# pashtari/factorizer

Measured on AMD Instinct MI355X. Metric: volumes/sec fwd+bwd, Swin Factorizer 128^3, higher is better.
Workload: dtype f32

## Files before the change

### factorizer_amd/_native.py

```python
from __future__ import annotations

import ctypes
import os
import threading

import torch

_HERE = os.path.dirname(os.path.abspath(__file__))
LIB_PATH = os.environ.get("FZ_LIB_PATH") or os.path.join(_HERE, "libfactorizer_hip.so")

FZ_OK = 0
FZ_E_UNSUPPORTED = -2
ABI_VERSION = 7
SOLVER_ID = {"mu": 0, "hals": 1, "cd": 2, "smu": 3}
STORE_F32, STORE_BF16 = 0, 1
PRODUCTS_DEFAULT, PRODUCTS_SPLIT_BF16, PRODUCTS_FP32_MFMA = 0, 1, 2
_products = threading.local()


def products() -> int:
    return getattr(_products, "value", PRODUCTS_DEFAULT)


class use_products:
# ... 163 lines not shown
    _fields_ = [("p", _vp), ("M", _i), ("pmul", _vp), ("pmul_kind", _i), ("q", _vp * 4), ("nsrc", _i),
                ("src_mode", _i), ("c0", _i), ("Cin", _i), ("K", _i), ("Vq", _i64), ("D", _i), ("H", _i),
                ("W", _i), ("N", _i64), ("Ho", _i), ("Wo", _i), ("stats", _vp), ("qact", _i), ("ln_g", _vp),
                ("ln_b", _vp), ("gw", _vp), ("gbias", _vp), ("accumulate", _i), ("B", _i), ("loader", _i),
                ("act_dtype", _i), ("products", _i)]


class VolGeom(_c.Structure):
    _fields_ = [("nd", _i), ("size", _i * 3), ("start", _i * 3), ("end", _i * 3), ("pad", _i * 3), ("out", _i * 3)]


class RespaceGeom(_c.Structure):
    _fields_ = [("nd", _i), ("src_size", _i * 3), ("src_axis", _i * 3), ("flip", _i * 3), ("res_size", _i * 3), ("pad", _i * 3),
                ("out", _i * 3), ("orig_size", _i * 3), ("box_start", _i * 3), ("scale", _c.c_double * 3),
                ("inv_scale", _c.c_double * 3)]


_SIGS.update({
    "fz_gcorr_supported": ([_i] * 5, _i),
    "fz_gcorr": ([_vp] * 5 + [_i] * 11 + [_f, _vp], _i),
    "fz_gcorr_wgrad_workspace_bytes": ([_i] * 10, _i64),
    "fz_gcorr_wgrad": ([_vp] * 4 + [_i] * 11 + [_vp], _i),
    "fz_gcorr_act": ([_vp] * 5 + [_i] * 11 + [_f, _i, _vp], _i),
    "fz_gcorr_wgrad_act": ([_vp] * 4 + [_i] * 12 + [_vp], _i),
    "fz_gcorr_mu_bwd": ([_vp] * 8 + [_i] * 11 + [_f, _i, _vp], _i),
    "fz_gnmf_supported": ([_i, _i64, _i, _i, _i], _i),
    "fz_gnmf_workspace_bytes": ([_i64, _i, _i64, _i, _i, _i], _i64),
    "fz_gnmf_launches": ([_i, _i, _i], _i),
    "fz_gnmf_fwd": ([_vp] * 6 + [_i64, _i, _i64, _i, _i, _i, _f, _vp, _vp], _i),
    "fz_gnmf_bwd": ([_vp] * 7 + [_i64, _i, _i64, _i, _i, _i, _i, _f, _vp, _vp], _i),
    "fz_nmf_cf_supported": ([_i] * 11, _i),
    "fz_nmf_cf_fwd": ([_vp] * 4 + [_i] * 5 + [_c.POINTER(_i)] + [_i] * 5 + [_f, _i, _vp], _i),
    "fz_nmf_cf_bwd": ([_vp] * 5 + [_i] * 5 + [_c.POINTER(_i)] + [_i] * 7 + [_f, _i, _vp], _i),
    "fz_nmf_cf_factors_supported": ([_i] * 12 + [_c.POINTER(_i)], _i),
    "fz_nmf_cf_fwd_store_factors": ([_vp] * 5 + [_i] * 5 + [_c.POINTER(_i)] + [_i] * 3 + [_f, _i, _vp], _i),
    "fz_nmf_cf_fwd_from_factors": ([_vp] * 6 + [_i] * 5 + [_c.POINTER(_i)] * 2 + [_i] * 4 + [_f, _i, _vp], _i),
    "fz_nmf_cf_bwd_factors_supported": ([_i] * 14 + [_c.POINTER(_i)], _i),
    "fz_nmf_cf_bwd_store_factors": ([_vp] * 5 + [_i] * 5 + [_c.POINTER(_i)] + [_i] * 3 + [_f, _i, _vp], _i),
    "fz_nmf_cf_bwd_from_factors": ([_vp] * 6 + [_i] * 5 + [_c.POINTER(_i)] * 2 + [_i] * 3 + [_f, _i, _vp], _i),
    "fz_nmf_pcf_supported": ([_i] * 11, _i),
    "fz_nmf_pcf_fwd": ([_vp] * 4 + [_i] * 8 + [_c.POINTER(_i)] + [_i] * 5 + [_f, _i, _vp], _i),
    "fz_nmf_pcf_bwd": ([_vp] * 5 + [_i] * 8 + [_c.POINTER(_i)] + [_i] * 7 + [_f, _i, _vp], _i),
    "fz_nmf_pcf_bwd_prefers_separate": ([_i] * 4, _i),
    "fz_act_add": ([_vp, _vp, _i64, _i, _vp], _i),
    "fz_mlp_pre_supported": ([_i, _i, _i64, _i], _i),
    "fz_mlp_drop_supported": ([_i, _i, _i64, _i], _i),
    "fz_mlp_chain_drop": ([_c.POINTER(MlpDesc), _c.POINTER(MlpDropout), _vp], _i),
    "fz_conv3_prologue_supported": ([_i] * 4, _i),
    "fz_conv3_fwd2": ([_vp] * 4 + [_i] * 8 + [_c.POINTER(BlockPrologue), _vp], _i),
    "fz_upcat2": ([_vp, _vp, _vp, _i, _vp, _vp, _vp] + [_i] * 7 + [_c.POINTER(BlockPrologue), _vp], _i),
    "fz_gemm": ([_c.POINTER(GemmDesc), _vp], _i),
    "fz_gemm_bx_enable": ([_i], _i),
    "fz_gemm_lnbwd_partials": ([_c.POINTER(GemmDesc)], _i64),
    "fz_reduce_rows": ([_vp, _i64, _i, _vp, _vp, _vp], _i),
    "fz_adamw_step": ([_vp, _vp, _vp, _vp, _i64, _f, _f, _f, _f, _f, _i, _f, _vp], _i),
    "fz_sw_gather": ([_vp, _vp] + [_i] * 10 + [_vp], _i),
    "fz_sw_accumulate": ([_vp] * 6 + [_f] + [_i] * 10 + [_vp], _i),
    "fz_sw_finalize": ([_vp, _vp, _i, _i64, _vp], _i),
    "fz_sw_gather2": ([_vp, _vp] + [_i] * 11 + [_vp], _i),
    "fz_sw_accumulate2": ([_vp] * 6 + [_f] + [_i] * 11 + [_vp], _i),
    "fz_sw_finalize2": ([_vp, _vp, _vp, _i, _i64, _i, _vp], _i),
    "fz_mlp_supported": ([_i, _i, _i64], _i),
    "fz_mlp_partials": ([_i, _i64], _i64),
    "fz_mlp_wgrad_rows": ([_i, _i64], _i),
    "fz_gemm_dw_rows": ([_i, _i64], _i),
    "fz_gemm_dw_workspace_bytes": ([_i, _i64], _i64),
    "fz_gemm_dw": ([_c.POINTER(GemmDwDesc), _vp], _i),
    "fz_mlp_wgrad_workspace_bytes": ([_i, _i64], _i64),
    "fz_mlp_chain": ([_c.POINTER(MlpDesc), _vp], _i),
    "fz_head_bwd_rows": ([], _i),
    "fz_head_bwd_workspace_bytes": ([], _i64),
    "fz_head_bwd": ([_vp, _vp, _vp, _vp, _vp, _i, _i, _i, _i64, _i, _vp], _i),
    "fz_head_fwd": ([_vp, _vp, _vp, _vp, _i, _i, _i, _i64, _i, _vp], _i),
    "fz_upcat_supported": ([_i] * 5, _i),
    "fz_upcat_compose": ([_vp, _vp, _i, _vp, _vp, _vp, _vp, _vp, _i, _i, _i, _vp], _i),
    "fz_upcat_wgrads": ([_vp, _vp, _vp, _i, _vp, _vp, _vp, _vp, _i, _vp, _i, _i, _i, _vp], _i),
    "fz_upcat": ([_vp, _vp, _vp, _i, _vp, _vp, _vp] + [_i] * 7 + [_vp], _i),
    "fz_upcat_bwd_supported": ([_i] * 6, _i),
    "fz_upcat_bwd_workspace_bytes": ([_i] * 4, _i64),
    "fz_upcat_bwd": ([_vp, _vp, _vp, _vp, _i, _vp, _vp, _vp, _vp, _vp, _i, _vp, _vp] + [_i] * 7 + [_vp], _i),
    "fz_wgrad": ([_c.POINTER(WgradDesc), _vp, _vp], _i),
    "fz_wgrad_group": ([_c.POINTER(_c.POINTER(WgradDesc)), _c.POINTER(_vp), _i, _vp], _i),
    "fz_wgrad_workspace_bytes": ([_c.POINTER(WgradDesc)], _i64),
    "fz_conv3_fwd": ([_vp] * 4 + [_i] * 8 + [_vp], _i),
    "fz_conv3_wgrad_chunks": ([_i] * 4, _i),
    "fz_conv3_wgrad_partials": ([_vp] * 4 + [_i] * 8 + [_vp], _i),
    "fz_chunk_reduce": ([_vp, _i, _i64, _vp, _i, _vp], _i),
    "fz_chunk_reduce_ld": ([_vp, _i, _i64, _i64, _vp, _i, _vp], _i),
    "fz_finish_defer": ([_i], _i),
    "fz_finish_pending": ([], _i),
    "fz_finish_flush": ([_vp], _i),
    "fz_finish_flush_all": ([_vp], _i),
    "fz_dice_bce_chunks": ([_i64], _i),
    "fz_dice_bce_sums": ([_vp, _vp, _vp, _i, _i64, _vp], _i),
    "fz_dice_bce_grad": ([_vp, _vp, _vp, _vp, _i, _i64, _f, _f, _vp, _vp], _i),
    "fz_dice_ce_sums": ([_vp, _vp, _vp, _i, _i, _i64, _vp], _i),
    "fz_dice_ce_grad": ([_vp, _vp, _vp, _vp, _i, _i, _i64, _f, _f, _vp, _vp], _i),
    "fz_dice_ce_finish": ([_vp, _i, _i, _i64, _f, _vp, _vp, _vp], _i),
    "fz_dice_bce_ds_sums": ([_vp, _vp, _vp, _i] + [_i] * 6 + [_i, _vp], _i),
    "fz_dice_bce_ds_grad": ([_vp, _vp, _vp, _vp, _i] + [_i] * 6 + [_i, _f, _f, _vp, _vp], _i),
    "fz_dice_ce_ds_sums": ([_vp, _vp, _vp, _i, _i] + [_i] * 6 + [_i, _vp], _i),
    "fz_dice_ce_ds_grad": ([_vp, _vp, _vp, _vp, _i, _i] + [_i] * 6 + [_i, _f, _f, _vp, _vp], _i),
    "fz_rowsum_chunks": ([_i64], _i),
    "fz_rowsum": ([_vp, _vp, _vp, _i, _i, _i64, _i, _vp], _i),
    "fz_ln_fwd": ([_vp] * 5 + [_i, _i, _i64, _f, _i, _vp], _i),
    "fz_ln_bwd": ([_vp] * 8 + [_i, _i, _i64, _i, _vp], _i),
    "fz_ln_bwd_workspace_bytes": ([_i], _i64),
    "fz_ln_bwd_workspace_bytes2": ([_i, _i, _i64], _i64),
    "fz_dropout_bits_words": ([_i, _i, _i64], _i64),
    "fz_dropout_keep_bits": ([_vp, _i, _i, _i, _i64, _f, _vp, _vp], _i),
    "fz_dropout_apply": ([_i, _vp, _f, _vp, _vp, _vp, _i, _i, _i64, _i, _vp], _i),
    "fz_seg_counts_chunks": ([_i64], _i),
    "fz_seg_counts_workspace_bytes": ([_i, _i64], _i64),
    "fz_seg_counts": ([_vp, _i, _vp, _i, _f, _vp, _vp, _vp, _i, _i64, _vp], _i),
    "fz_mask_edges": ([_vp, _vp, _vp, _i, _i, _i, _i, _i, _vp], _i),
    "fz_edge_min_dist2_splits": ([_i64, _i64], _i),
    "fz_edge_min_dist2_workspace_bytes": ([_i64, _i64], _i64),
    "fz_edge_min_dist2": ([_vp, _i64, _vp, _i64, _f, _f, _f, _vp, _vp, _vp], _i),
    "fz_aug_record_floats": ([], _i),
    "fz_aug_resample": ([_vp, _vp, _i, _i, _vp, _vp, _i, _vp, _vp, _vp] + [_i] * 6 + [_vp], _i),
    "fz_aug_smooth": ([_vp, _vp, _i, _i, _vp, _vp] + [_i] * 6 + [_vp], _i),
    "fz_aug_noise_field": ([_vp, _vp, _i, _i, _i64, _vp], _i),
    "fz_aug_source_words": ([], _i),
    "fz_aug_crop_resample": ([_vp, _vp, _i, _i, _vp, _i, _vp, _vp, _vp] + [_i] * 6 + [_vp], _i),
    "fz_vol_kind_ok": ([_i, _i], _i),
    "fz_vol_bbox": ([_vp, _i, _i, _i, _i, _i, _i, _vp, _vp], _i),
    "fz_vol_workspace_bytes": ([_i, _c.POINTER(VolGeom)], _i64),
    "fz_vol_stats": ([_vp, _i, _i, _c.POINTER(VolGeom), _i, _i, _vp, _vp], _i),
    "fz_vol_write": ([_vp, _i, _vp, _i, _i, _vp, _i, _i, _c.POINTER(_i), _c.POINTER(_i), _i, _vp, _c.POINTER(VolGeom), _i, _i,
                      _vp, _vp, _vp, _vp], _i),
    "fz_vol_restore": ([_c.POINTER(_vp), _i, _i, _i, _c.POINTER(VolGeom), _f, _c.POINTER(_c.c_ubyte), _vp, _vp], _i),
    "fz_vol_respace": ([_vp, _i, _vp, _i, _vp, _i, _vp, _c.POINTER(RespaceGeom), _i, _vp], _i),
    "fz_vol_unspace": ([_c.POINTER(_vp), _i, _i, _i, _c.POINTER(RespaceGeom), _i, _i, _f, _vp, _vp], _i),
    "fz_inorm_one_pass_max": ([], _i),
    "fz_inorm_chunks": ([_i64], _i),
    "fz_inorm_workspace_bytes": ([_i64, _i64], _i64),
    "fz_inorm_fwd": ([_vp] * 5 + [_i64, _i, _i64, _c.c_double, _i, _vp, _vp], _i),
    "fz_inorm_bwd": ([_vp] * 7 + [_i64, _i, _i64, _i, _vp, _vp], _i),
})
SEG_F32, SEG_BF16, SEG_U8 = 0, 1, 2
VOL_F32, VOL_BF16, VOL_U8, VOL_I16 = 0, 1, 2, 3
VOL_IMAGE_IN, VOL_IMAGE_OUT, VOL_LABEL_IN, VOL_LOGITS = 0, 1, 2, 3
RESPACE_BILINEAR, RESPACE_NEAREST = 0, 1
DROP_RES, DROP_GELU, DROP_GELU_BWD = 0, 1, 2
```

### factorizer_amd/csrc/wgrad.hip

```cpp
#include <type_traits>

#include "fz_common.h"
#include "finish.h"

namespace fz {

typedef float f32x16 __attribute__((ext_vector_type(16)));
typedef float f32x2 __attribute__((ext_vector_type(2)));
typedef __bf16 bf16x2 __attribute__((ext_vector_type(2)));
typedef __bf16 bf16x8 __attribute__((ext_vector_type(8)));

__device__ __forceinline__ void split_bf16x8(const float (&x)[8], bf16x8& hi, bf16x8& mid, bf16x8& lo) {
#pragma unroll
  for (int e = 0; e < 8; e += 2) {
    const f32x2 v = {x[e], x[e + 1]};
    const bf16x2 h2 = __builtin_convertvector(v, bf16x2);
    const f32x2 r = v - __builtin_convertvector(h2, f32x2);
    const bf16x2 m2 = __builtin_convertvector(r, bf16x2);
    const f32x2 r2 = r - __builtin_convertvector(m2, f32x2);
    const bf16x2 l2 = __builtin_convertvector(r2, bf16x2);
    hi[e] = h2[0]; hi[e + 1] = h2[1];
    mid[e] = m2[0]; mid[e + 1] = m2[1];
    lo[e] = l2[0]; lo[e + 1] = l2[1];
  }
// ... 262 lines not shown
    for (int i = 0; i < MBP; ++i) {
      float s = psum[i] + __shfl_xor(psum[i], 32, 64);
      if (h == 0) red[wave * 32 + c] = s;
      __syncthreads();
      if (threadIdx.x < 32) {
        const float tot = (red[threadIdx.x] + red[32 + threadIdx.x]) + (red[64 + threadIdx.x] + red[96 + threadIdx.x]);
        const int m = m0 + i * 32 + threadIdx.x;
        if (m < a.M) a.part_bias[(int64_t)blockIdx.x * a.M + m] = tot;
      }
      __syncthreads();
    }
  }
}

enum { QP_NONE = 0, QP_STATS = 1, QP_GELU = 2, QP_RELU = 3 };
constexpr int kStrideF = 36;

template <int MBP, int MBQ, int QPRO, int BF, typename AT>
__device__ __forceinline__ void wgrad_fast_body(const WgradArgsT<AT>& a, float* lds, const int bx, const int by, const int bz) {
#define WG_BX bx
#define WG_BY by
#define WG_BZ bz
#include "wgrad_fast_body.inc"
#undef WG_BX
#undef WG_BY
#undef WG_BZ
}

template <int MBP, int MBQ, int QPRO, int BF = 0, typename AT = float>
__global__ __launch_bounds__(256, 2) void wgrad_fast_kernel(WgradArgsT<AT> a) {
  extern __shared__ __attribute__((aligned(16))) float lds[];
#define WG_BX blockIdx.x
#define WG_BY blockIdx.y
#define WG_BZ blockIdx.z
#include "wgrad_fast_body.inc"
#undef WG_BX
#undef WG_BY
#undef WG_BZ
}

constexpr int kWgGroupMax = 4;
template <typename AT>
struct WgradGroupT {
  WgradArgsT<AT> a[kWgGroupMax];
  int start[kWgGroupMax + 1];
  int gx[kWgGroupMax], gy[kWgGroupMax];
  int qpro[kWgGroupMax];
  int n;
};

template <int MBP, int MBQ, int BF, typename AT>
__global__ __launch_bounds__(256, 2) void wgrad_fast_group_kernel(WgradGroupT<AT> g) {
  extern __shared__ __attribute__((aligned(16))) float lds[];
  int i = 0;
#pragma unroll
  for (int t = 1; t < kWgGroupMax; ++t)
    if (t < g.n && (int)blockIdx.x >= g.start[t]) i = t;
  int local = (int)blockIdx.x - g.start[i];
  const int bx = local % g.gx[i];
  local /= g.gx[i];
  const int by = local % g.gy[i], bz = local / g.gy[i];
  const WgradArgsT<AT>& a = g.a[i];
  switch (g.qpro[i]) {
    case QP_STATS: wgrad_fast_body<MBP, MBQ, QP_STATS, BF, AT>(a, lds, bx, by, bz); break;
    case QP_GELU: wgrad_fast_body<MBP, MBQ, QP_GELU, BF, AT>(a, lds, bx, by, bz); break;
    case QP_RELU: wgrad_fast_body<MBP, MBQ, QP_RELU, BF, AT>(a, lds, bx, by, bz); break;
    default: wgrad_fast_body<MBP, MBQ, QP_NONE, BF, AT>(a, lds, bx, by, bz); break;
  }
}


__global__ __launch_bounds__(256) void ln_fold_kernel(float* __restrict__ gw, const float* __restrict__ acc,
                                                      const float* __restrict__ gb, const float* __restrict__ ln_g,
                                                      const float* __restrict__ ln_b, int M, int K, int accumulate) {
  const int64_t e = (int64_t)blockIdx.x * blockDim.x + threadIdx.x;
  if (e >= (int64_t)M * K) return;
  const int m = (int)(e / K), k = (int)(e % K);
  const float v = ln_g[k] * acc[e] + ln_b[k] * gb[m];
  gw[e] = accumulate ? gw[e] + v : v;
}

}

using namespace fz;

static bool use_fast(const fz_wgrad_desc* d) {
  const int PR = d->M > 32 ? 64 : 32, QR = d->K > 32 ? 64 : 32;
  const int c0 = d->c0 > 0 ? d->c0 : d->Cin;
  bool fast = PR == 64 && QR == 64 && d->loader == QL_PLAIN && !d->pmul && (d->M % PR) == 0 && (d->K % QR) == 0 &&
              (d->N % kTile) == 0 && d->N == d->Vq && (c0 % 8) == 0 && d->src_mode == 0 && !(d->stats && d->qact) &&
              (int64_t)8 * d->N < ((int64_t)1 << 30);
  { const auto& k = FZ_KNOB("FZ_WGRAD_FAST"); if (k.set && k.val == 0) fast = false; }
  return fast;
}

static int pick_chunks(int64_t total_tiles, int out_blocks, bool fast, int* tiles_per_chunk) {
  int64_t total_units = fast ? 1024 : 2048;
  int64_t units_target = total_units / (out_blocks > 0 ? out_blocks : 1);
  if (units_target < 16) units_target = 16;
  int64_t tpc = (total_tiles + units_target - 1) / units_target;
  if (tpc < 1) tpc = 1;
  *tiles_per_chunk = (int)tpc;
  int64_t units = (total_tiles + tpc - 1) / tpc;
  return (int)((units + 3) / 4);
}

extern "C" int64_t fz_wgrad_workspace_bytes(const fz_wgrad_desc* d) {
  if (!d || d->M < 1 || d->K < 1) return -1;
  const int PR = d->M > 32 ? 64 : 32, QR = d->K > 32 ? 64 : 32;
  const int out_blocks = ((d->M + PR - 1) / PR) * ((d->K + QR - 1) / QR);
  const int64_t total_tiles = ((d->N + kTile - 1) / kTile) * d->B;
  int tpc;
  const int nchunk = pick_chunks(total_tiles, out_blocks, use_fast(d), &tpc);
  return ((int64_t)nchunk * d->M * d->K + (int64_t)nchunk * d->M + (int64_t)d->M * d->K + d->M) *
         (int64_t)sizeof(float);
}

static bool fz_wgrad_group_enabled() {
  const bool v = !(FZ_KNOB("FZ_WGRAD_GROUP").set && FZ_KNOB("FZ_WGRAD_GROUP").val == 0);
  return v;
}

template <typename AT>
struct WgradPlan {
  WgradArgsT<AT> a;
  dim3 grid;
  int PR, QR, nchunk, qp;
  bool fast;
};

template <typename AT>
static int wgrad_plan(const fz_wgrad_desc* d, void* workspace, WgradPlan<AT>& pl) {
  if (!d->p || !d->q[0] || !d->gw) return fail(FZ_E_ARG, "fz_wgrad: null pointer");
  if (d->loader < 0 || d->loader > QL_K3_2D) return fail(FZ_E_ARG, "fz_wgrad: bad loader");
  if ((d->loader == QL_S2D_2D || d->loader == QL_K3_2D) && (d->nsrc != 1 || d->src_mode != 0 || d->stats || d->qact))
    return fail(FZ_E_ARG, "fz_wgrad: a 2-D loader takes one source and no Q prologue");
  if (d->loader == QL_S2D_2D && (d->K != 4 * d->Cin || (d->Wo & 1) || d->Ho < 1 || d->Wo < 1 || d->H != 2 * d->Ho ||
                                 d->W != 2 * d->Wo || d->N != (int64_t)d->Ho * d->Wo || d->Vq != (int64_t)d->H * d->W))
    return fail(FZ_E_SHAPE, "fz_wgrad: 2-D s2d shape (K = 4*Cin, (H, W) = 2*(Ho, Wo), even Wo, N = Ho*Wo)");
  if (d->loader == QL_K3_2D && (d->K != 9 * d->Cin || d->H < 1 || d->W < 1 || d->N != (int64_t)d->H * d->W || d->Vq != d->N))
    return fail(FZ_E_SHAPE, "fz_wgrad: 2-D k3 shape (K = 9*Cin, N = Vq = H*W)");
  if (d->N % 4 != 0) return fail(FZ_E_UNSUPPORTED, "fz_wgrad: column count must be a multiple of 4");
  if (d->loader == QL_S2D && ((d->Wo & 1) || d->K != 8 * d->Cin)) return fail(FZ_E_SHAPE, "fz_wgrad: s2d shape");
  if (d->loader == QL_K3 && d->K != 27 * d->Cin) return fail(FZ_E_SHAPE, "fz_wgrad: k3 shape");
  const int PR = d->M > 32 ? 64 : 32, QR = d->K > 32 ? 64 : 32;
  const int gy = (d->M + PR - 1) / PR, gz = (d->K + QR - 1) / QR;
  const int64_t total_tiles = ((d->N + kTile - 1) / kTile) * d->B;
  int tpc;
  pl.fast = use_fast(d);
  pl.PR = PR; pl.QR = QR;
  pl.nchunk = pick_chunks(total_tiles, gy * gz, pl.fast, &tpc);
  pl.qp = d->stats ? QP_STATS : (d->qact == 2 ? QP_GELU : (d->qact == 1 ? QP_RELU : QP_NONE));
  WgradArgsT<AT>& a = pl.a;
  a.p = (const AT*)d->p; a.M = d->M; a.pmul = (const AT*)d->pmul; a.pmul_kind = d->pmul_kind;
  for (int i = 0; i < 4; ++i) a.q[i] = (const AT*)d->q[i];
  a.nsrc = d->nsrc; a.src_mode = d->src_mode; a.c0 = d->c0 > 0 ? d->c0 : d->Cin; a.Cin = d->Cin; a.K = d->K;
  a.Vq = d->Vq; a.D = d->D; a.H = d->H; a.W = d->W; a.N = d->N; a.Ho = d->Ho; a.Wo = d->Wo;
  if (d->loader == QL_S2D_2D || d->loader == QL_K3_2D) a.D = 1;
  a.stats = d->stats; a.qact = d->qact; a.B = d->B; a.tiles_per_chunk = tpc;
  a.part = (float*)workspace;
  a.part_bias = a.part + (int64_t)pl.nchunk * d->M * d->K;
  pl.grid = dim3(pl.nchunk, gy, gz);
  return FZ_OK;
}

static size_t wgrad_fast_lds(int PR, int QR) {
  const size_t ldsf = (size_t)4 * (PR + QR) * kStrideF * sizeof(float);
  const size_t ldsr = (size_t)4 * 1024 * sizeof(float);
  return ldsf > ldsr ? ldsf : ldsr;
}

template <typename AT>
static int wgrad_main_launch(const fz_wgrad_desc* d, const WgradPlan<AT>& pl, hipStream_t st) {
  const WgradArgsT<AT>& a = pl.a;
  const int PR = pl.PR, QR = pl.QR;
  const dim3 grid = pl.grid, block(256);
  const size_t lds = (size_t)4 * (PR + QR) * kStride * sizeof(float);
  constexpr bool kBf16 = !std::is_same<AT, float>::value;
  const int bf3g = products_split(d->products);
#define FZ_WG(MBP, MBQ, QL)                                                                        \
  do {                                                                                             \
    if (kBf16) hipLaunchKernelGGL((wgrad_kernel<MBP, MBQ, QL, 1>), grid, block, lds, st, a);       \
    else if (bf3g) hipLaunchKernelGGL((wgrad_kernel<MBP, MBQ, QL, 6>), grid, block, lds, st, a);   \
    else hipLaunchKernelGGL((wgrad_kernel<MBP, MBQ, QL, 0>), grid, block, lds, st, a);             \
  } while (0)
#define FZ_WG_SHAPES(QL)                                 \
  do {                                                   \
    if (PR == 64 && QR == 64) FZ_WG(2, 2, QL);           \
    else if (PR == 64) FZ_WG(2, 1, QL);                  \
    else if (QR == 64) FZ_WG(1, 2, QL);                  \
    else FZ_WG(1, 1, QL);                                \
  } while (0)
  if (pl.fast) {
    const int qp = pl.qp;
    const size_t ldsz = wgrad_fast_lds(PR, QR);
    const int bf3 = bf3g;
#define FZ_WGF(MBP, MBQ, QP)                                                                              \
  do {                                                                                                    \
    if (kBf16) hipLaunchKernelGGL((wgrad_fast_kernel<MBP, MBQ, QP, 1>), grid, block, ldsz, st, a);        \
    else if (bf3) hipLaunchKernelGGL((wgrad_fast_kernel<MBP, MBQ, QP, 6>), grid, block, ldsz, st, a);     \
    else hipLaunchKernelGGL((wgrad_fast_kernel<MBP, MBQ, QP, 0>), grid, block, ldsz, st, a);              \
  } while (0)
#define FZ_WGF_SHAPES(QP)                                \
  do {                                                   \
    if (PR == 64 && QR == 64) FZ_WGF(2, 2, QP);          \
    else if (PR == 64) FZ_WGF(2, 1, QP);                 \
    else if (QR == 64) FZ_WGF(1, 2, QP);                 \
    else FZ_WGF(1, 1, QP);                               \
  } while (0)
    if (qp == QP_STATS) FZ_WGF_SHAPES(QP_STATS);
    else if (qp == QP_GELU) FZ_WGF_SHAPES(QP_GELU);
    else if (qp == QP_RELU) FZ_WGF_SHAPES(QP_RELU);
    else FZ_WGF_SHAPES(QP_NONE);
  } else if (d->loader == QL_PLAIN) FZ_WG_SHAPES(QL_PLAIN);
  else if (d->loader == QL_S2D) FZ_WG_SHAPES(QL_S2D);
  else if (d->loader == QL_S2D_2D) FZ_WG_SHAPES(QL_S2D_2D);
  else if (d->loader == QL_K3_2D) FZ_WG_SHAPES(QL_K3_2D);
  else FZ_WG_SHAPES(QL_K3);
  FZ_LAUNCH_CHECK();
  return FZ_OK;
}

template <typename AT>
static FinishJob wgrad_finish_job(const fz_wgrad_desc* d, const WgradPlan<AT>& pl) {
  const int64_t MK = (int64_t)d->M * d->K;
  int wide = (pl.nchunk <= 64 && MK >= 16384) ? 1 : ((pl.nchunk <= 256 && MK >= 4096) ? 2 : 0);
  auto al16 = [](const void* q) { return (reinterpret_cast<uintptr_t>(q) & 15) == 0; };
  if (wide == 1 && MK >= 65536 && (d->M % 4) == 0 && (d->K % 4) == 0 && al16(pl.a.part) && al16(d->gw) &&
      (d->gbias == nullptr || (al16(pl.a.part_bias) && al16(d->gbias))) && (d->ln_g == nullptr || (al16(d->ln_g) && al16(d->ln_b))))
    wide = 3;
  const int per = wide == 3 ? 1024 : (wide == 1 ? 256 : (wide == 2 ? 64 : 8));
  const int nbw = (int)((MK + per - 1) / per);
  const int nbb = d->gbias != nullptr ? (d->M + per - 1) / per : 0;
  FinishJob j = finish_job(FK_WGRAD, nbw + nbb);
  j.u.wg = WgradFinishOne{pl.a.part, pl.a.part_bias, d->gw, d->gbias, d->ln_g != nullptr ? d->ln_g : (const float*)nullptr, d->ln_b,
                          pl.nchunk, d->M, d->K, d->accumulate, nbw, wide};
  return j;
}
template <typename AT>
static int wgrad_finish_launch(const fz_wgrad_desc* d, const WgradPlan<AT>& pl, hipStream_t st) {
  const FinishJob j = wgrad_finish_job<AT>(d, pl);
  return finish_run(&j, 1, st);
}

template <typename AT>
static int wgrad_launch(const fz_wgrad_desc* d, void* workspace, fz_stream_t stream) {
  WgradPlan<AT> pl;
  const int rc = wgrad_plan<AT>(d, workspace, pl);
  if (rc != FZ_OK) return rc;
  if (d->B == 0) return FZ_OK;
  const int rc2 = wgrad_main_launch<AT>(d, pl, (hipStream_t)stream);
  if (rc2 != FZ_OK) return rc2;
  return wgrad_finish_launch<AT>(d, pl, (hipStream_t)stream);
}

template <typename AT>
static int wgrad_group_launch(const fz_wgrad_desc* const* ds, void* const* ws, int n, fz_stream_t stream) {
  WgradPlan<AT> pl[kWgGroupMax];
  bool groupable = n >= 2 && fz_wgrad_group_enabled();
  for (int i = 0; i < n; ++i) {
    const int rc = wgrad_plan<AT>(ds[i], ws[i], pl[i]);
    if (rc != FZ_OK) return rc;
    groupable = groupable && pl[i].fast && pl[i].PR == 64 && pl[i].QR == 64 && ds[i]->B > 0 &&
                products_split(ds[i]->products) == products_split(ds[0]->products);
  }
  hipStream_t st = (hipStream_t)stream;
  if (!groupable) {
    for (int i = 0; i < n; ++i) {
      if (ds[i]->B == 0) continue;
      int rc = wgrad_main_launch<AT>(ds[i], pl[i], st);
      if (rc == FZ_OK) rc = wgrad_finish_launch<AT>(ds[i], pl[i], st);
      if (rc != FZ_OK) return rc;
    }
    return FZ_OK;
  }
  WgradGroupT<AT> g;
  int total = 0;
  for (int i = 0; i < kWgGroupMax; ++i) {
    const int j = i < n ? i : n - 1;
    g.a[i] = pl[j].a;
    g.start[i] = total;
    g.gx[i] = (int)pl[j].grid.x; g.gy[i] = (int)pl[j].grid.y;
    g.qpro[i] = pl[j].qp;
    if (i < n) total += (int)(pl[i].grid.x * pl[i].grid.y * pl[i].grid.z);
  }
  g.start[kWgGroupMax] = total;
  g.n = n;
  const size_t ldsz = wgrad_fast_lds(64, 64);
  constexpr bool kBf16 = !std::is_same<AT, float>::value;
  const int bf3 = products_split(ds[0]->products);
  if (kBf16) hipLaunchKernelGGL((wgrad_fast_group_kernel<2, 2, 1, AT>), dim3(total), dim3(256), ldsz, st, g);
  else if (bf3) hipLaunchKernelGGL((wgrad_fast_group_kernel<2, 2, 6, AT>), dim3(total), dim3(256), ldsz, st, g);
  else hipLaunchKernelGGL((wgrad_fast_group_kernel<2, 2, 0, AT>), dim3(total), dim3(256), ldsz, st, g);
  FZ_LAUNCH_CHECK();
  FinishJob fj[kWgGroupMax];
  for (int i = 0; i < n; ++i) fj[i] = wgrad_finish_job<AT>(ds[i], pl[i]);
  return finish_run(fj, n, st);
}

extern "C" int fz_wgrad(const fz_wgrad_desc* d, void* workspace, fz_stream_t stream) {
  if (!d || !workspace) return fail(FZ_E_ARG, "fz_wgrad: null descriptor/workspace");
  if (d->act_dtype == FZ_STORE_F32) return wgrad_launch<float>(d, workspace, stream);
  if (d->act_dtype == FZ_STORE_BF16) return wgrad_launch<bf16>(d, workspace, stream);
  return fail(FZ_E_ARG, "fz_wgrad: act_dtype must be FZ_STORE_F32 or FZ_STORE_BF16");
}

extern "C" int fz_wgrad_group(const fz_wgrad_desc* const* descs, void* const* workspaces, int n, fz_stream_t stream) {
  if (!descs || !workspaces || n < 1 || n > kWgGroupMax) return fail(FZ_E_ARG, "fz_wgrad_group: 1..4 descriptors");
  for (int i = 0; i < n; ++i) {
    if (!descs[i] || !workspaces[i]) return fail(FZ_E_ARG, "fz_wgrad_group: null descriptor/workspace");
    if (descs[i]->act_dtype != descs[0]->act_dtype) return fail(FZ_E_ARG, "fz_wgrad_group: one activation storage type per group");
  }
  if (descs[0]->act_dtype == FZ_STORE_F32) return wgrad_group_launch<float>(descs, workspaces, n, stream);
  if (descs[0]->act_dtype == FZ_STORE_BF16) return wgrad_group_launch<bf16>(descs, workspaces, n, stream);
  return fail(FZ_E_ARG, "fz_wgrad_group: act_dtype must be FZ_STORE_F32 or FZ_STORE_BF16");
}

extern "C" int fz_chunk_reduce_ld(const float* part, int nchunk, int64_t n, int64_t ld, float* out, int accumulate,
                                  fz_stream_t stream) {
  if (!part || !out || nchunk < 1 || n < 1 || ld < n) return fail(FZ_E_ARG, "fz_chunk_reduce: bad arguments");
  FinishJob j = finish_job(FK_CHUNK, (int)((n + 7) / 8));
  j.u.chunk = FinChunk{part, out, (long long)n, (long long)ld, nchunk, accumulate};
  return finish_run(&j, 1, (hipStream_t)stream);
}

extern "C" int fz_chunk_reduce(const float* part, int nchunk, int64_t n, float* out, int accumulate,
                               fz_stream_t stream) {
  return fz_chunk_reduce_ld(part, nchunk, n, n, out, accumulate, stream);
}
```

### include/factorizer_hip.h

```cpp
#ifndef FACTORIZER_HIP_H
#define FACTORIZER_HIP_H

#include <stdint.h>

#ifdef __cplusplus
extern "C" {
#endif

#define FZ_OK 0
#define FZ_E_SHAPE (-1)
#define FZ_E_UNSUPPORTED (-2)
#define FZ_E_HIP (-3)
#define FZ_E_ARG (-4)

#define FZ_STORE_F32 0
#define FZ_STORE_BF16 1

#define FZ_SOLVER_MU 0
#define FZ_SOLVER_HALS 1
#define FZ_SOLVER_CD 2
#define FZ_SOLVER_SMU 3

typedef void* fz_stream_t;

// ... 199 lines not shown
  int ldgw;
  int ldw;
  const uint32_t* drop_m;
  float drop_s;
} fz_gemm_dw_desc;
int fz_gemm_dw_rows(int B, int64_t V);
int64_t fz_gemm_dw_workspace_bytes(int B, int64_t V);
int fz_gemm_dw(const fz_gemm_dw_desc* desc, fz_stream_t stream);

int fz_head_bwd_rows(void);
int64_t fz_head_bwd_workspace_bytes(void);
int fz_head_bwd(const void* gy, const void* x, const float* w, void* gx, float* part, int B, int M, int C, int64_t V,
                int act_dtype, fz_stream_t stream);
int fz_head_fwd(const void* x, const float* w, const float* bias, void* y, int B, int M, int C, int64_t V, int act_dtype,
                fz_stream_t stream);

int fz_upcat_compose(const float* w_t, const float* w_b, int ldb, const float* b_t, const float* b_ad, float* wc, float* wbt, float* bias,
                     int Cd, int O, int M, fz_stream_t stream);
int fz_upcat_wgrads(const float* gt, const float* w_t, const float* w_b, int ldb, const float* gb_ad, const float* b_t, float* gw_t,
                    float* gw_b, int ldg, float* gb_t, int Cd, int O, int M, fz_stream_t stream);
int fz_upcat_supported(int C, int Cd, int D, int H, int W);
int fz_upcat(const void* skip, const void* deep, const float* wa, int lda, const float* wbt, const float* bias, void* out,
             int B, int C, int Cd, int D, int H, int W, int act_dtype, fz_stream_t stream);
int fz_upcat_bwd_supported(int C1, int Cd, int D, int H, int W, int act_dtype);
int64_t fz_upcat_bwd_workspace_bytes(int B, int D, int H, int W);
int fz_upcat_bwd(const void* g, const void* skip, const void* deep, const float* wa, int lda, const float* wc, void* g_skip,
                 void* g_deep, void* workspace, float* gw_a, int ldg, float* gb, float* gt, int B, int C1, int Cd, int D, int H,
                 int W, int act_dtype, fz_stream_t stream);
typedef struct fz_block_prologue {
  const float* ln_g;
  const float* ln_b;
  float ln_eps;
  const float* w;
  void* t;
  float* stats;
} fz_block_prologue;
int fz_upcat2(const void* skip, const void* deep, const float* wa, int lda, const float* wbt, const float* bias, void* out,
              int B, int C, int Cd, int D, int H, int W, int act_dtype, const fz_block_prologue* pro, fz_stream_t stream);

int fz_mlp_supported(int C, int H, int64_t V);
int fz_mlp_pre_supported(int C, int H, int64_t V, int products);
int fz_mlp_drop_supported(int C, int H, int64_t V, int products);
int64_t fz_mlp_partials(int B, int64_t V);
int fz_mlp_wgrad_rows(int B, int64_t V);
int64_t fz_mlp_wgrad_workspace_bytes(int B, int64_t V);
int fz_mlp_chain(const fz_mlp_desc* desc, fz_stream_t stream);
int fz_mlp_chain_drop(const fz_mlp_desc* desc, const fz_mlp_dropout* drop, fz_stream_t stream);

#define FZ_QL_PLAIN 0
#define FZ_QL_S2D 1
#define FZ_QL_K3 2
#define FZ_QL_S2D_2D 3
#define FZ_QL_K3_2D 4

typedef struct fz_wgrad_desc {
  const void* p;
  int M;
  const void* pmul;
  int pmul_kind;
  const void* q[4];
  int nsrc, src_mode, c0;
  int Cin;
  int K;
  int64_t Vq;
  int D, H, W;
  int64_t N;
  int Ho, Wo;
  const float* stats;
  int qact;
  const float* ln_g;
  const float* ln_b;
  float* gw;
  float* gbias;
  int accumulate;
  int B;
  int loader;
  int act_dtype;
  int products;
} fz_wgrad_desc;

int64_t fz_wgrad_workspace_bytes(const fz_wgrad_desc* desc);
int fz_wgrad(const fz_wgrad_desc* desc, void* workspace, fz_stream_t stream);
int fz_wgrad_group(const fz_wgrad_desc* const* descs, void* const* workspaces, int n, fz_stream_t stream);

int fz_ln_fwd(const void* x , const float* gamma, const float* beta, void* y ,
              float* stats, int B, int C, int64_t V, float eps, int act_dtype, fz_stream_t stream);
int64_t fz_ln_bwd_workspace_bytes(int C);
int64_t fz_ln_bwd_workspace_bytes2(int B, int C, int64_t V);
int fz_ln_bwd(const void* gl, const void* x, const float* stats, const float* gamma,
              const void* gadd, void* gx , float* gparams, void* workspace,
              int B, int C, int64_t V, int act_dtype, fz_stream_t stream);

int fz_conv3_fwd(const void* x , const float* w, const float* bias, void* y ,
                 int B, int Cin, int M, int D, int H, int W, int act_dtype, int products, fz_stream_t stream);
struct fz_block_prologue;
int fz_conv3_prologue_supported(int Cin, int M, int W, int products);
int fz_conv3_fwd2(const void* x, const float* w, const float* bias, void* y, int B, int Cin, int M, int D, int H, int W,
                  int act_dtype, int products, const struct fz_block_prologue* pro, fz_stream_t stream);
int fz_conv3_wgrad_chunks(int B, int D, int H, int W);
int fz_conv3_wgrad_partials(const void* gy, const void* x , float* part, float* part_bias, int B,
                            int Cin, int M, int D, int H, int W, int act_dtype, int products, fz_stream_t stream);
int fz_chunk_reduce(const float* part, int nchunk, int64_t n, float* out, int accumulate, fz_stream_t stream);
int fz_chunk_reduce_ld(const float* part, int nchunk, int64_t n, int64_t ld, float* out, int accumulate, fz_stream_t stream);

int fz_rowsum_chunks(int64_t V);
int fz_rowsum(const void* x , float* part, float* out, int B, int C, int64_t V, int act_dtype,
              fz_stream_t stream);

int fz_gcorr_supported(int Ci, int Co, int kd, int kh, int kw);
int fz_gcorr(const float* in, const float* w, float* out, const float* mul_a, const float* mul_b, int B, int G,
             int Ci, int Co, int D, int H, int W, int kd, int kh, int kw, int w_batched, float add_eps,
             fz_stream_t stream);
int64_t fz_gcorr_wgrad_workspace_bytes(int B, int G, int Ci, int Co, int D, int H, int W, int kd, int kh, int kw);
int fz_gcorr_wgrad(const float* in, const float* gout, float* gw, void* ws, int B, int G, int Ci, int Co, int D, int H,
                   int W, int kd, int kh, int kw, int w_batched, fz_stream_t stream);
int fz_gcorr_act(const void* in, const float* w, void* out, const void* mul_a, const void* mul_b, int B, int G,
                 int Ci, int Co, int D, int H, int W, int kd, int kh, int kw, int w_batched, float add_eps,
                 int act_dtype, fz_stream_t stream);
int fz_gcorr_wgrad_act(const void* in, const void* gout, float* gw, void* ws, int B, int G, int Ci, int Co, int D, int H,
                       int W, int kd, int kh, int kw, int w_batched, int act_dtype, fz_stream_t stream);
int fz_gcorr_mu_bwd(const void* r, const float* wT, const void* g, const void* s, const void* num, void* ds, void* dnum,
                    void* dden, int B, int G, int Ci, int Co, int D, int H, int W, int kd, int kh, int kw, int w_batched,
                    float eps, int act_dtype, fz_stream_t stream);

int fz_dice_bce_chunks(int64_t V);
int fz_dice_bce_sums(const float* z, const float* t, float* part, int planes, int64_t V, fz_stream_t stream);
int fz_dice_bce_grad(const float* z, const float* t, const float* coef, float* gz, int planes, int64_t V,
                     float cd, float cb, const float* gscale, fz_stream_t stream);

int fz_dice_ce_sums(const float* z, const float* t, float* part, int B, int C, int64_t V, fz_stream_t stream);
int fz_dice_ce_finish(const float* part, int B, int C, int64_t V, float smooth, float* loss, float* coef, fz_stream_t stream);
int fz_dice_ce_grad(const float* z, const float* t, const float* coef, float* gz, int B, int C, int64_t V,
                    float cd, float cb, const float* gscale, fz_stream_t stream);

int fz_dice_bce_ds_sums(const float* z, const void* t, float* part, int planes, int Td, int Th, int Tw, int Ld, int Lh, int Lw,
                        int tkind, fz_stream_t stream);
int fz_dice_bce_ds_grad(const float* z, const void* t, const float* coef, float* gz, int planes, int Td, int Th, int Tw,
                        int Ld, int Lh, int Lw, int tkind, float cd, float cb, const float* gscale, fz_stream_t stream);
int fz_dice_ce_ds_sums(const float* z, const void* t, float* part, int B, int C, int Td, int Th, int Tw, int Ld, int Lh, int Lw,
                       int tkind, fz_stream_t stream);
int fz_dice_ce_ds_grad(const float* z, const void* t, const float* coef, float* gz, int B, int C, int Td, int Th, int Tw,
                       int Ld, int Lh, int Lw, int tkind, float cd, float cb, const float* gscale, fz_stream_t stream);

int fz_sw_gather(const float* vol, float* win, int C, int D, int H, int W, int rd, int rh, int rw, int z0, int y0,
                 int x0, fz_stream_t stream);
int fz_sw_accumulate(const float* prob, float* out, float* cnt, const float* gz, const float* gy, const float* gx,
                     float wmin, int C, int D, int H, int W, int rd, int rh, int rw, int z0, int y0, int x0,
                     fz_stream_t stream);
int fz_sw_finalize(float* out, const float* cnt, int C, int64_t V, fz_stream_t stream);
int fz_sw_gather2(const void* img, void* win, int C, int D, int H, int W, int rd, int rh, int rw, int z0, int y0, int x0,
                  int act_dtype, fz_stream_t stream);
int fz_sw_accumulate2(const void* prob, float* out, float* cnt, const float* gz, const float* gy, const float* gx,
                      float wmin, int C, int D, int H, int W, int rd, int rh, int rw, int z0, int y0, int x0, int act_dtype,
                      fz_stream_t stream);
int fz_sw_finalize2(const float* out, const float* cnt, void* res, int C, int64_t V, int act_dtype, fz_stream_t stream);

#define FZ_SEG_F32 0
#define FZ_SEG_BF16 1
#define FZ_SEG_U8 2
int fz_seg_counts_chunks(int64_t V);
int64_t fz_seg_counts_workspace_bytes(int planes, int64_t V);
int fz_seg_counts(const void* pred, int pred_kind, const void* label, int label_kind, float bound, uint8_t* mask,
                  void* workspace, int64_t* counts, int planes, int64_t V, fz_stream_t stream);
int fz_mask_edges(const uint8_t* mask, uint8_t* edges, int64_t* counts, int planes, int nd, int D, int H, int W,
                  fz_stream_t stream);
int fz_edge_min_dist2_splits(int64_t nq, int64_t nt);
// ... 88 lines not shown
```

Before: 133.7.

## Add 128x128 tiled split-bf16 MFMA weight-gradient kernel with grouped launch

Adds a new weight-gradient kernel for f32 activations with split-bf16 products. Each workgroup owns a 128x128 output tile and loops over a strided set of N-slabs. P and Q are split into three bf16 levels in swizzled LDS, loads for the next slab are prefetched into registers, and each level pair is accumulated with 32x32x16 MFMAs. It covers plain and space-to-depth loaders, has a grouped multi-descriptor variant, and adds a query for which kernel is selected. The aim is more output reuse per workgroup and fewer partial chunks than the 64x64 fast path, at the cost of a large LDS footprint and more registers.

```diff
diff --git a/factorizer_amd/_native.py b/factorizer_amd/_native.py
--- a/factorizer_amd/_native.py
+++ b/factorizer_amd/_native.py
@@ -269,6 +269,7 @@
     "fz_wgrad": ([_c.POINTER(WgradDesc), _vp, _vp], _i),
     "fz_wgrad_group": ([_c.POINTER(_c.POINTER(WgradDesc)), _c.POINTER(_vp), _i, _vp], _i),
     "fz_wgrad_workspace_bytes": ([_c.POINTER(WgradDesc)], _i64),
+    "fz_wgrad_kernel_kind": ([_c.POINTER(WgradDesc)], _i),
     "fz_conv3_fwd": ([_vp] * 4 + [_i] * 8 + [_vp], _i),
     "fz_conv3_wgrad_chunks": ([_i] * 4, _i),
     "fz_conv3_wgrad_partials": ([_vp] * 4 + [_i] * 8 + [_vp], _i),
diff --git a/factorizer_amd/csrc/wgrad.hip b/factorizer_amd/csrc/wgrad.hip
--- a/factorizer_amd/csrc/wgrad.hip
+++ b/factorizer_amd/csrc/wgrad.hip
@@ -368,6 +368,8 @@
 
 }
 
+#include "wgrad_tile.h"
+
 using namespace fz;
 
 static bool use_fast(const fz_wgrad_desc* d) {
@@ -391,15 +393,64 @@
   return (int)((units + 3) / 4);
 }
 
+static bool use_tile(const fz_wgrad_desc* d) {
+  if (d->act_dtype != FZ_STORE_F32 || !products_split(d->products) || d->pmul || d->B < 1) return false;
+  if (d->M < kWtSide || d->K < kWtSide || (d->M % kWtSide) != 0 || (d->K % kWtSide) != 0) return false;
+  if (d->N < kTile || (d->N % kTile) != 0 || d->N >= ((int64_t)1 << 31) || (d->N / kTile) * d->B >= ((int64_t)1 << 31)) return false;
+  if (d->src_mode != 0 || (d->stats && d->qact)) return false;
+  { const auto& k = FZ_KNOB("FZ_WGRAD_TILE"); if (k.set && k.val == 0) return false; }
+  if (d->loader == QL_PLAIN) {
+    const int64_t cols = d->N * d->B;
+    if (cols >= 2048 && cols < 16384) return false;
+    const int c0 = d->c0 > 0 ? d->c0 : d->Cin;
+    return d->N == d->Vq && d->K == d->Cin && (c0 % 8) == 0 && c0 <= d->Cin && (c0 == d->Cin || d->q[1] != nullptr);
+  }
+  if (d->loader == QL_S2D)
+    return d->nsrc == 1 && !d->stats && !d->qact && d->K == 8 * d->Cin && d->Ho >= 1 && d->Wo >= 2 && (d->Wo & 1) == 0 &&
+           d->H == 2 * d->Ho && d->W == 2 * d->Wo && d->Vq == 8 * d->N && d->Vq < ((int64_t)1 << 31) && (d->N % ((int64_t)d->Ho * d->Wo)) == 0;
+  return false;
+}
+
+static int pick_tile_chunks(int64_t total_slabs, int tiles, int* slabs_per_chunk) {
+  int wgs = 512, min_slabs = 8, max_chunks = 128;
+  { const auto& k = FZ_KNOB("FZ_WGRAD_TILE_WGS"); if (k.set && k.val > 0) wgs = k.val; }
+  { const auto& k = FZ_KNOB("FZ_WGRAD_TILE_SLABS"); if (k.set && k.val > 0) min_slabs = k.val; }
+  { const auto& k = FZ_KNOB("FZ_WGRAD_TILE_CHUNKS"); if (k.set && k.val > 0) max_chunks = k.val; }
+  int64_t want = (wgs + tiles - 1) / tiles;
+  if (want > max_chunks) want = max_chunks;
+  if (want > total_slabs / min_slabs) want = total_slabs / min_slabs;
+  if (want < 1) want = 1;
+  const int64_t spc = (total_slabs + want - 1) / want;
+  *slabs_per_chunk = (int)spc;
+  return (int)((total_slabs + spc - 1) / spc);
+}
+
+enum { WK_GENERIC = 0, WK_FAST = 1, WK_TILE = 2 };
+static int wgrad_kind_chunks(const fz_wgrad_desc* d, int* nchunk, int* tiles_per_chunk) {
+  const int64_t total_tiles = ((d->N + kTile - 1) / kTile) * d->B;
+  if (use_tile(d)) {
+    *nchunk = pick_tile_chunks(total_tiles, (d->M / kWtSide) * (d->K / kWtSide), tiles_per_chunk);
+    return WK_TILE;
+  }
+  const int PR = d->M > 32 ? 64 : 32, QR = d->K > 32 ? 64 : 32;
+  const int out_blocks = ((d->M + PR - 1) / PR) * ((d->K + QR - 1) / QR);
+  const bool fast = use_fast(d);
+  *nchunk = pick_chunks(total_tiles, out_blocks, fast, tiles_per_chunk);
+  return fast ? WK_FAST : WK_GENERIC;
+}
+
 extern "C" int64_t fz_wgrad_workspace_bytes(const fz_wgrad_desc* d) {
   if (!d || d->M < 1 || d->K < 1) return -1;
-  const int PR = d->M > 32 ? 64 : 32, QR = d->K > 32 ? 64 : 32;
-  const int out_blocks = ((d->M + PR - 1) / PR) * ((d->K + QR - 1) / QR);
-  const int64_t total_tiles = ((d->N + kTile - 1) / kTile) * d->B;
-  int tpc;
-  const int nchunk = pick_chunks(total_tiles, out_blocks, use_fast(d), &tpc);
+  int nchunk, tpc;
+  wgrad_kind_chunks(d, &nchunk, &tpc);
   return ((int64_t)nchunk * d->M * d->K + (int64_t)nchunk * d->M + (int64_t)d->M * d->K + d->M) *
          (int64_t)sizeof(float);
+}
+
+extern "C" int fz_wgrad_kernel_kind(const fz_wgrad_desc* d) {
+  if (!d || d->M < 1 || d->K < 1) return -1;
+  int nchunk, tpc;
+  return wgrad_kind_chunks(d, &nchunk, &tpc);
 }
 
 static bool fz_wgrad_group_enabled() {
@@ -412,7 +463,7 @@
   WgradArgsT<AT> a;
   dim3 grid;
   int PR, QR, nchunk, qp;
-  bool fast;
+  bool fast, tile;
 };
 
 template <typename AT>
@@ -431,11 +482,11 @@
   if (d->loader == QL_K3 && d->K != 27 * d->Cin) return fail(FZ_E_SHAPE, "fz_wgrad: k3 shape");
   const int PR = d->M > 32 ? 64 : 32, QR = d->K > 32 ? 64 : 32;
   const int gy = (d->M + PR - 1) / PR, gz = (d->K + QR - 1) / QR;
-  const int64_t total_tiles = ((d->N + kTile - 1) / kTile) * d->B;
   int tpc;
-  pl.fast = use_fast(d);
+  const int kind = wgrad_kind_chunks(d, &pl.nchunk, &tpc);
+  pl.fast = kind == WK_FAST;
+  pl.tile = kind == WK_TILE;
   pl.PR = PR; pl.QR = QR;
-  pl.nchunk = pick_chunks(total_tiles, gy * gz, pl.fast, &tpc);
   pl.qp = d->stats ? QP_STATS : (d->qact == 2 ? QP_GELU : (d->qact == 1 ? QP_RELU : QP_NONE));
   WgradArgsT<AT>& a = pl.a;
   a.p = (const AT*)d->p; a.M = d->M; a.pmul = (const AT*)d->pmul; a.pmul_kind = d->pmul_kind;
@@ -446,7 +497,7 @@
   a.stats = d->stats; a.qact = d->qact; a.B = d->B; a.tiles_per_chunk = tpc;
   a.part = (float*)workspace;
   a.part_bias = a.part + (int64_t)pl.nchunk * d->M * d->K;
-  pl.grid = dim3(pl.nchunk, gy, gz);
+  pl.grid = pl.tile ? dim3(pl.nchunk * (d->M / kWtSide) * (d->K / kWtSide)) : dim3(pl.nchunk, gy, gz);
   return FZ_OK;
 }
 
@@ -477,6 +528,18 @@
     else if (QR == 64) FZ_WG(1, 2, QL);                  \
     else FZ_WG(1, 1, QL);                                \
   } while (0)
+  if constexpr (!kBf16) {
+    if (pl.tile) {
+      const size_t ldst = kWtLds;
+      if (d->loader == QL_S2D) hipLaunchKernelGGL((wgrad_tile_kernel<QL_S2D, QP_NONE>), grid, block, ldst, st, a);
+      else if (pl.qp == QP_STATS) hipLaunchKernelGGL((wgrad_tile_kernel<QL_PLAIN, QP_STATS>), grid, block, ldst, st, a);
+      else if (pl.qp == QP_GELU) hipLaunchKernelGGL((wgrad_tile_kernel<QL_PLAIN, QP_GELU>), grid, block, ldst, st, a);
+      else if (pl.qp == QP_RELU) hipLaunchKernelGGL((wgrad_tile_kernel<QL_PLAIN, QP_RELU>), grid, block, ldst, st, a);
+      else hipLaunchKernelGGL((wgrad_tile_kernel<QL_PLAIN, QP_NONE>), grid, block, ldst, st, a);
+      FZ_LAUNCH_CHECK();
+      return FZ_OK;
+    }
+  }
   if (pl.fast) {
     const int qp = pl.qp;
     const size_t ldsz = wgrad_fast_lds(PR, QR);
@@ -544,13 +607,35 @@
 static int wgrad_group_launch(const fz_wgrad_desc* const* ds, void* const* ws, int n, fz_stream_t stream) {
   WgradPlan<AT> pl[kWgGroupMax];
   bool groupable = n >= 2 && fz_wgrad_group_enabled();
+  bool tiled = groupable;
   for (int i = 0; i < n; ++i) {
     const int rc = wgrad_plan<AT>(ds[i], ws[i], pl[i]);
     if (rc != FZ_OK) return rc;
+    tiled = tiled && pl[i].tile && ds[i]->loader == QL_PLAIN;
     groupable = groupable && pl[i].fast && pl[i].PR == 64 && pl[i].QR == 64 && ds[i]->B > 0 &&
                 products_split(ds[i]->products) == products_split(ds[0]->products);
   }
   hipStream_t st = (hipStream_t)stream;
+  if constexpr (std::is_same<AT, float>::value) {
+    if (tiled) {
+      WgradTileGroup g;
+      int total = 0;
+      for (int i = 0; i < kWgGroupMax; ++i) {
+        const int j = i < n ? i : n - 1;
+        g.a[i] = pl[j].a;
+        g.start[i] = total;
+        g.qpro[i] = pl[j].qp;
+        if (i < n) total += (int)pl[i].grid.x;
+      }
+      g.start[kWgGroupMax] = total;
+      g.n = n;
+      hipLaunchKernelGGL(wgrad_tile_group_kernel, dim3(total), dim3(256), (size_t)kWtLds, st, g);
+      FZ_LAUNCH_CHECK();
+      FinishJob fj[kWgGroupMax];
+      for (int i = 0; i < n; ++i) fj[i] = wgrad_finish_job<AT>(ds[i], pl[i]);
+      return finish_run(fj, n, st);
+    }
+  }
   if (!groupable) {
     for (int i = 0; i < n; ++i) {
       if (ds[i]->B == 0) continue;
diff --git a/factorizer_amd/csrc/wgrad_tile.h b/factorizer_amd/csrc/wgrad_tile.h
--- /dev/null
+++ b/factorizer_amd/csrc/wgrad_tile.h
@@ -0,0 +1,200 @@
+#pragma once
+
+namespace fz {
+
+typedef __bf16 bf16x4 __attribute__((ext_vector_type(4)));
+
+constexpr int kWtSide = 128;
+constexpr int kWtLevel = 2 * kWtSide * 64;
+constexpr int kWtLds = 3 * kWtLevel;
+
+__device__ __forceinline__ int wt_off(int row, int ch) { return row * 64 + ((ch ^ ((row >> 2) & 3)) << 4); }
+
+__device__ __forceinline__ void wt_split_store(char* lds, int row, int cq, float x0, float x1, float x2, float x3) {
+  const f32x2 va = {x0, x1}, vb = {x2, x3};
+  const bf16x2 ha = __builtin_convertvector(va, bf16x2), hb = __builtin_convertvector(vb, bf16x2);
+  const f32x2 ra = va - __builtin_convertvector(ha, f32x2), rb = vb - __builtin_convertvector(hb, f32x2);
+  const bf16x2 ma = __builtin_convertvector(ra, bf16x2), mb = __builtin_convertvector(rb, bf16x2);
+  const f32x2 sa = ra - __builtin_convertvector(ma, f32x2), sb = rb - __builtin_convertvector(mb, f32x2);
+  const bf16x2 la = __builtin_convertvector(sa, bf16x2), lb = __builtin_convertvector(sb, bf16x2);
+  char* d = lds + wt_off(row, cq >> 1) + (cq & 1) * 8;
+  *reinterpret_cast<bf16x4*>(d) = bf16x4{ha[0], ha[1], hb[0], hb[1]};
+  *reinterpret_cast<bf16x4*>(d + kWtLevel) = bf16x4{ma[0], ma[1], mb[0], mb[1]};
+  *reinterpret_cast<bf16x4*>(d + 2 * kWtLevel) = bf16x4{la[0], la[1], lb[0], lb[1]};
+}
+
+constexpr int QP_RUNTIME = -1;
+template <int QL, int QPRO>
+__device__ __forceinline__ void wgrad_tile_body(const WgradArgsT<float>& a, char* lds, const int chunk, const int tm, const int tk,
+                                                const int qpro_rt = QP_NONE) {
+  const int qp = QPRO == QP_RUNTIME ? qpro_rt : QPRO;
+  const int tid = threadIdx.x, lane = tid & 63, wave = tid >> 6;
+  const int m0 = tm * kWtSide, k0 = tk * kWtSide;
+  const int sps = (int)(a.N / kTile);
+  const int total = sps * a.B;
+  const int nchunk = (total + a.tiles_per_chunk - 1) / a.tiles_per_chunk;
+  const int s_begin = chunk, s_end = total;
+
+  f32x16 acc[2][2], cor[2][2];
+#pragma unroll
+  for (int i = 0; i < 2; ++i)
+#pragma unroll
+    for (int j = 0; j < 2; ++j)
+#pragma unroll
+      for (int r = 0; r < 16; ++r) acc[i][j][r] = cor[i][j][r] = 0.f;
+  float psum[4] = {0.f, 0.f, 0.f, 0.f};
+
+  const int cq = tid & 7, r0 = tid >> 3;
+  float4 pv[4], qv[4], mu4, rs4;
+
+  auto issue_loads = [&](int s) {
+    const int b = s / sps;
+    const int64_t n0 = (int64_t)(s - b * sps) * kTile;
+    const float* pb = a.p + ((int64_t)b * a.M + m0 + r0) * a.N + n0 + cq * 4;
+#pragma unroll
+    for (int i = 0; i < 4; ++i) pv[i] = ld4(pb + (int64_t)(32 * i) * a.N);
+    if (QL == QL_PLAIN) {
+#pragma unroll
+      for (int i = 0; i < 4; ++i) {
+        const int k = k0 + r0 + 32 * i;
+        const bool first = k < a.c0;
+        const float* base = first ? a.q[0] : a.q[1];
+        const int cs = first ? a.c0 : a.Cin - a.c0;
+        const int ci = first ? k : k - a.c0;
+        qv[i] = ld4(base + ((int64_t)b * cs + ci) * a.Vq + n0 + cq * 4);
+      }
+      if (qp == QP_STATS) {
+        const float* st = a.stats + (int64_t)b * 2 * a.Vq + n0 + cq * 4;
+        mu4 = ld4(st);
+        rs4 = ld4(st + a.Vq);
+      }
+    } else {
+      unsigned col[2];
+#pragma unroll
+      for (int j = 0; j < 2; ++j) {
+        const unsigned n = (unsigned)n0 + 4u * cq + 2u * j;
+        const unsigned wo = n % (unsigned)a.Wo, t2 = n / (unsigned)a.Wo;
+        const unsigned ho = t2 % (unsigned)a.Ho, dz = t2 / (unsigned)a.Ho;
+        col[j] = ((2 * dz) * (unsigned)a.H + 2 * ho) * (unsigned)a.W + 2 * wo;
+      }
+#pragma unroll
+      for (int i = 0; i < 4; ++i) {
+        const int k = k0 + 2 * (r0 + 32 * (i >> 1));
+        const int ci = k >> 3, td = (k >> 2) & 1, th = (k >> 1) & 1;
+        qv[i] = ld4(a.q[0] + ((int64_t)b * a.Cin + ci) * a.Vq + ((unsigned)(td * a.H + th) * (unsigned)a.W + col[i & 1]));
+      }
+    }
+  };
+
+  const int c = lane & 31, h = lane >> 5;
+  const int wm = wave >> 1, wk = wave & 1;
+
+  if (s_begin < s_end) issue_loads(s_begin);
+  for (int s = s_begin; s < s_end; s += nchunk) {
+#pragma unroll
+    for (int i = 0; i < 4; ++i) {
+      psum[i] += (pv[i].x + pv[i].y) + (pv[i].z + pv[i].w);
+      wt_split_store(lds, r0 + 32 * i, cq, pv[i].x, pv[i].y, pv[i].z, pv[i].w);
+    }
+    if (QL == QL_PLAIN) {
+#pragma unroll
+      for (int i = 0; i < 4; ++i) {
+        float4 v = qv[i];
+        if (qp == QP_STATS) {
+          v.x = (v.x - mu4.x) * rs4.x; v.y = (v.y - mu4.y) * rs4.y; v.z = (v.z - mu4.z) * rs4.z; v.w = (v.w - mu4.w) * rs4.w;
+        } else if (qp == QP_GELU) {
+          v.x = gelu_w(v.x); v.y = gelu_w(v.y); v.z = gelu_w(v.z); v.w = gelu_w(v.w);
+        } else if (qp == QP_RELU) {
+          v.x = fmaxf(v.x, 0.f); v.y = fmaxf(v.y, 0.f); v.z = fmaxf(v.z, 0.f); v.w = fmaxf(v.w, 0.f);
+        }
+        wt_split_store(lds, kWtSide + r0 + 32 * i, cq, v.x, v.y, v.z, v.w);
+      }
+    } else {
+#pragma unroll
+      for (int rp = 0; rp < 2; ++rp) {
+        const int row = kWtSide + 2 * (r0 + 32 * rp);
+        const float4 u = qv[2 * rp], w = qv[2 * rp + 1];
+        wt_split_store(lds, row, cq, u.x, u.z, w.x, w.z);
+        wt_split_store(lds, row + 1, cq, u.y, u.w, w.y, w.w);
+      }
+    }
+    __syncthreads();
+    if (s + nchunk < s_end) issue_loads(s + nchunk);
+#pragma unroll
+    for (int t = 0; t < 2; ++t) {
+#pragma unroll
+      for (int j = 0; j < 2; ++j) {
+        const char* src = lds + wt_off(kWtSide + wk * 64 + j * 32 + c, 2 * t + h);
+        const bf16x8 qh = *reinterpret_cast<const bf16x8*>(src);
+        const bf16x8 qm = *reinterpret_cast<const bf16x8*>(src + kWtLevel);
+        const bf16x8 ql = *reinterpret_cast<const bf16x8*>(src + 2 * kWtLevel);
+#pragma unroll
+        for (int i = 0; i < 2; ++i) {
+          int poff = wt_off(wm * 64 + i * 32 + c, 2 * t + h);
+          asm volatile("" : "+v"(poff));
+          const bf16x8 ph = *reinterpret_cast<const bf16x8*>(lds + poff);
+          const bf16x8 pm = *reinterpret_cast<const bf16x8*>(lds + poff + kWtLevel);
+          const bf16x8 pl = *reinterpret_cast<const bf16x8*>(lds + poff + 2 * kWtLevel);
+          cor[i][j] = __builtin_amdgcn_mfma_f32_32x32x16_bf16(pl, qh, cor[i][j], 0, 0, 0);
+          cor[i][j] = __builtin_amdgcn_mfma_f32_32x32x16_bf16(pm, qm, cor[i][j], 0, 0, 0);
+          cor[i][j] = __builtin_amdgcn_mfma_f32_32x32x16_bf16(ph, ql, cor[i][j], 0, 0, 0);
+          cor[i][j] = __builtin_amdgcn_mfma_f32_32x32x16_bf16(pm, qh, cor[i][j], 0, 0, 0);
+          cor[i][j] = __builtin_amdgcn_mfma_f32_32x32x16_bf16(ph, qm, cor[i][j], 0, 0, 0);
+          acc[i][j] = __builtin_amdgcn_mfma_f32_32x32x16_bf16(ph, qh, acc[i][j], 0, 0, 0);
+        }
+      }
+    }
+    __syncthreads();
+  }
+
+  float* part = a.part + ((int64_t)chunk * a.M + m0 + wm * 64) * a.K + k0 + wk * 64 + c;
+#pragma unroll
+  for (int i = 0; i < 2; ++i)
+#pragma unroll
+    for (int j = 0; j < 2; ++j)
+#pragma unroll
+      for (int r = 0; r < 16; ++r) {
+        const int row = i * 32 + (r & 3) + 8 * (r >> 2) + 4 * h;
+        part[(int64_t)row * a.K + j * 32] = acc[i][j][r] + cor[i][j][r];
+      }
+  if (a.part_bias != nullptr && tk == 0) {
+#pragma unroll
+    for (int i = 0; i < 4; ++i) {
+      float sum = psum[i];
+      sum += __shfl_xor(sum, 1, 64);
+      sum += __shfl_xor(sum, 2, 64);
+      sum += __shfl_xor(sum, 4, 64);
+      if (cq == 0) a.part_bias[(int64_t)chunk * a.M + m0 + r0 + 32 * i] = sum;
+    }
+  }
+}
+
+template <int QL, int QPRO>
+__global__ __launch_bounds__(256, 2) void wgrad_tile_kernel(WgradArgsT<float> a) {
+  extern __shared__ __attribute__((aligned(16))) float lds[];
+  const int ntk = a.K / kWtSide, tiles = (a.M / kWtSide) * ntk;
+  const int tile = (int)blockIdx.x % tiles, chunk = (int)blockIdx.x / tiles;
+  wgrad_tile_body<QL, QPRO>(a, reinterpret_cast<char*>(lds), chunk, tile / ntk, tile % ntk);
+}
+
+struct WgradTileGroup {
+  WgradArgsT<float> a[4];
+  int start[5];
+  int qpro[4];
+  int n;
+};
+
+__global__ __launch_bounds__(256, 2) void wgrad_tile_group_kernel(WgradTileGroup g) {
+  extern __shared__ __attribute__((aligned(16))) float lds[];
+  int i = 0;
+#pragma unroll
+  for (int t = 1; t < 4; ++t)
+    if (t < g.n && (int)blockIdx.x >= g.start[t]) i = t;
+  const WgradArgsT<float>& a = g.a[i];
+  const int local = (int)blockIdx.x - g.start[i];
+  const int ntk = a.K / kWtSide, tiles = (a.M / kWtSide) * ntk;
+  const int tile = local % tiles, chunk = local / tiles;
+  wgrad_tile_body<QL_PLAIN, QP_RUNTIME>(a, reinterpret_cast<char*>(lds), chunk, tile / ntk, tile % ntk, g.qpro[i]);
+}
+
+}
diff --git a/include/factorizer_hip.h b/include/factorizer_hip.h
--- a/include/factorizer_hip.h
+++ b/include/factorizer_hip.h
@@ -305,6 +305,10 @@
 int64_t fz_wgrad_workspace_bytes(const fz_wgrad_desc* desc);
 int fz_wgrad(const fz_wgrad_desc* desc, void* workspace, fz_stream_t stream);
 int fz_wgrad_group(const fz_wgrad_desc* const* descs, void* const* workspaces, int n, fz_stream_t stream);
+#define FZ_WGRAD_KERNEL_GENERIC 0
+#define FZ_WGRAD_KERNEL_FAST 1
+#define FZ_WGRAD_KERNEL_TILE 2
+int fz_wgrad_kernel_kind(const fz_wgrad_desc* desc);
 
 int fz_ln_fwd(const void* x , const float* gamma, const float* beta, void* y ,
               float* stats, int B, int C, int64_t V, float eps, int act_dtype, fz_stream_t stream);
```

New measurement: 133.2. About the same (-0.4%).
